# NJU-LHRS/LHRS-Bot

Hardware: AMD Instinct MI355X
Metric: stage-1 pretrain samples/sec (224^2 image + 128-tok caption) (higher is better)
Workload: dtype bf16

## Files before the change

include/lhrs_hip.h:

```cpp
#ifndef LHRS_HIP_H
#define LHRS_HIP_H
#include <stdint.h>
#ifdef __cplusplus
extern "C" {
#endif

typedef uint16_t lhrs_bf16_t;

const char* lhrs_last_error(void);
int lhrs_abi_version(void);
const char* lhrs_target_arch(void);

int lhrs_gemm_bf16_nt(const void* A, int lda, const void* B, int ldb, void* C, int ldc, int M, int N, int K,
                      const void* bias, const void* residual, int ldr, int act, int out_f32, int accumulate,
                      float alpha, void* stream);

int lhrs_gemm_bf16_nt_lora(const void* A, int lda, const void* B, int ldb, const void* A2, int lda2, const void* B2, int ldb2,
                           int K2, void* C, int ldc, int M, int N, int K, const void* bias, const void* residual, int ldr,
                           int out_f32, int accumulate, float alpha, void* stream);
int lhrs_gemm_fp8_nt(const void* A8, long lda, const float* sa, const void* B8, long ldb, const float* sb, void* C, int ldc,
                     int M, int N, int K, const void* residual, int ldr, float alpha, void* stream);
int lhrs_gemm_fp8_nt_lora(const void* A8, long lda, const float* sa, const void* B8, long ldb, const float* sb, const void* A2,
                          int lda2, const void* B2, int ldb2, int K2, void* C, int ldc, int M, int N, int K,
                          const void* residual, int ldr, float alpha, void* stream);
// ... 52 lines not shown
int lhrs_gemm_u4_nt(const void* A, int lda, const void* B, int ldb, void* C, int ldc, int M, int N, int K, const void* residual, int ldr,
                    void* stream);
int lhrs_gemm_u4_nt_lora(const void* A, int lda, const void* B, int ldb, const void* A2, int lda2, const void* B2, int ldb2, int K2, void* C, int ldc,
                         int M, int N, int K, const void* residual, int ldr, void* stream);
int lhrs_gemm_u4_fused_takes(int kind, int M, int tiles_n, int K, int K2);
int lhrs_gemm_u4_main_rows(int M, int N);
int lhrs_gemm_u4_rope(const void* X, int ldx, const void* W, int ldw, void* C, int ldc, int M, int N, int K, const float* cos_t,
                      const float* sin_t, int pos_mod, int pos0, int rope_cols, void* stream);
int lhrs_gemm_u4_rope_lora(const void* X, int ldx, const void* W, int ldw, const void* A2, int lda2, const void* B2, int ldb2, int K2, void* C, int ldc,
                           int M, int N, int K, const float* cos_t, const float* sin_t, int pos_mod, int pos0, int rope_cols, void* stream);
int lhrs_gemm_u4_swiglu_fwd(const void* X, int ldx, const void* Wgu, int ldw, void* gu, int ld_gu, void* act, int ld_act, int M, int ff, int K,
                            void* stream);
int lhrs_gemm_u4_swiglu_bwd(const void* dY, int ldy, const void* WdT, int ldw, const void* gu, void* dgu, int ld_gu, int M, int ff, int K,
                            void* stream);

int lhrs_tn_skinny_splits(int M, int N);
int lhrs_gemm_tn_skinny(const void* P, long ldp, const void* Q, long ldq, float* C, long ldc, float* partial, int M, int N,
                        int KP, int accumulate, void* stream);
int lhrs_blockdiag_mask(float* g, long ld, int rows, int cols, int r, int w, int active_mask, void* stream);

int lhrs_layernorm_fwd(const void* x, long ldx, const void* gamma, const void* beta, void* y, long ldy, float* mean,
                       float* rstd, int rows, int cols, float eps, void* stream);
int lhrs_layernorm_bwd_nblk(int rows);
int lhrs_layernorm_bwd(const void* dy, long ld_dy, const void* x, long ldx, const void* gamma, const float* mean,
                       const float* rstd, const void* add, void* dx, long ld_dx, float* dgamma, float* dbeta,
                       float* partial, int accumulate, int rows, int cols, void* stream);
int lhrs_rmsnorm_fwd(const void* x, long ldx, const void* w, void* y, long ldy, float* rstd, int rows, int cols,
                     float eps, void* stream);
int lhrs_rmsnorm_bwd(const void* dy, const void* x, const void* w, const float* rstd, const void* add, void* dx,
                     int rows, int cols, float eps, void* stream);

int lhrs_seq_transpose(const void* in, long ld_in, void* out, int cols, int LT, const int* desc, int nseq, int use_kv,
                       void* stream);
int lhrs_attn_fwd(const void* q, long ldq, const void* k, long ldk, const void* v, long ldv, void* o, long ldo, float* lse,
                  const int* desc, int nseq, int H, int D, int max_q, int max_kv, int LTq, int causal, float scale,
                  void* stream);
int lhrs_attn_fwd_kmask(const void* q, long ldq, const void* k, long ldk, const void* v, long ldv, void* o, long ldo,
                        float* lse, const int* desc, int nseq, int H, int D, int max_q, int max_kv, int LTq,
                        int causal, float scale, const unsigned char* key_mask, long ld_mask, void* stream);
int lhrs_attn_delta(const void* o, long ldo, const void* dout, long ld_do, float* delta, const int* desc, int nseq, int H,
                    int D, int max_q, int LTq, void* stream);
int lhrs_attn_bwd(const void* q, long ldq, const void* k, long ldk, const void* v, long ldv, const void* dout,
                  long ld_do, const float* lse, const float* delta, void* dq, long ld_dq, void* dk, long ld_dk, void* dv,
                  long ld_dv, const int* desc, int nseq, int H, int D, int max_q, int max_kv, int LTq, int causal,
                  float scale, void* stream);
int lhrs_attn_bwd_rope(const void* q, long ldq, const void* k, long ldk, const void* v, long ldv, const void* dout,
                       long ld_do, const float* lse, const float* delta, void* dq, long ld_dq, void* dk, long ld_dk, void* dv,
                       long ld_dv, const int* desc, int nseq, int H, int D, int max_q, int max_kv, int LTq, int causal,
                       float scale, const float* cos_t, const float* sin_t, int pos_mod, int pos0, long rows, void* stream);
int lhrs_attn_bwd_o(const void* q, long ldq, const void* k, long ldk, const void* v, long ldv, const void* dout, long ld_do,
                    const void* o, long ldo, const float* lse, float* delta, void* dq, long ld_dq, void* dk, long ld_dk, void* dv,
                    long ld_dv, const int* desc, int nseq, int H, int D, int max_q, int max_kv, int LTq, int causal, float scale,
                    const float* cos_t, const float* sin_t, int pos_mod, int pos0, long rows, void* stream);

int lhrs_patchify(const float* rgb, void* out, int B, int img, int P, int KP, void* stream);
int lhrs_vit_assemble(const void* patch, const void* cls, const void* pos, void* out, int B, int NP, int dim,
                      void* stream);
int lhrs_rope(void* x, long ld, int rows, int nheads, int D, const float* cos_t, const float* sin_t, const int* pos_ids,
              int pos_mod, int pos0, int inverse, void* stream);
int lhrs_swiglu_fwd(const void* gate_up, void* act, long rows, int F, void* stream);
int lhrs_swiglu_bwd(const void* dact, const void* gate_up, void* dgate_up, long rows, int F, void* stream);
int lhrs_map(int op, const void* a, const void* b, void* out, long n, void* stream);
int lhrs_colsum_nsplit(int rows);
int lhrs_colsum(const void* x, long ld, float* out, float* partial, int rows, int cols, int accumulate, void* stream);
int lhrs_cast_f32_to_bf16(const float* in, void* out, long n, void* stream);
int lhrs_cast_bf16_to_f32(const void* in, float* out, long n, void* stream);
// ... 98 lines not shown
```

lhrs_bot_amd/csrc/attention.hip:

```cpp
#include "common.h"
#include <type_traits>

namespace {

struct AttnArgs {
  const bf16_t* q; const bf16_t* k; const bf16_t* v; const bf16_t* dout;
  long ldq, ldk, ldv, ldo, ld_do, ld_dq, ld_dk, ld_dv;
  bf16_t* o; bf16_t* dq; bf16_t* dk; bf16_t* dv;
  int LTq;
  float* lse;
  const float* delta;
  const int* desc;
  int H;
  float scale;
  const unsigned char* kmask;
  long ld_kmask;
  const float* rope_cos;
  const float* rope_sin;
  int rope_mod, rope_pos0;
  const bf16_t* o_in;
  long ld_oin;
  float* delta_w;
  int wide;
};

constexpr float NEG_INF = -__builtin_huge_valf();

template <int D>
__device__ __forceinline__ int swz(int row) {
  return D == 128 ? (((row & 7) << 1) | ((row >> 3) & 1)) : (row & 7);
}
template <int D>
__device__ __forceinline__ int rm_off(int row, int c) { return row * (D * 2) + ((c ^ swz<D>(row)) << 4); }

template <int D> struct TileRegs { uint4 v[64 * (D / 8) / 256]; };

template <int D>
__device__ __forceinline__ void tile_load(TileRegs<D>& r, const bf16_t* base, long ld, int row0, int len, int tid) {
  constexpr int CH = D / 8, N = 64 * CH / 256;
#pragma unroll
  for (int i = 0; i < N; ++i) {
    const int idx = tid + i * 256;
    const int gr = min(row0 + idx / CH, len - 1);
    r.v[i] = *reinterpret_cast<const uint4*>(base + (long)gr * ld + (idx % CH) * 8);
  }
}
template <int D>
__device__ __forceinline__ void tile_store(char* lds, const TileRegs<D>& r, int tid) {
  constexpr int CH = D / 8, N = 64 * CH / 256;
#pragma unroll
  for (int i = 0; i < N; ++i) {
    const int idx = tid + i * 256;
    *reinterpret_cast<uint4*>(lds + rm_off<D>(idx / CH, idx % CH)) = r.v[i];
  }
}
template <int D>
// ... 382 lines not shown
#pragma unroll
    for (int db = 0; db < DB; ++db) dk[db] = MFMA(join(blo[db], bhi[db]), d0, dk[db]);
    tr_wait<DB>(alo, ahi);
    tr_issue<D, 1>(tq, blo, bhi);
    __builtin_amdgcn_sched_barrier(0);
#pragma unroll
    for (int db = 0; db < DB; ++db) dv[db] = MFMA(join(alo[db], ahi[db]), p1, dv[db]);
    tr_wait<DB>(blo, bhi);
#pragma unroll
    for (int db = 0; db < DB; ++db) dk[db] = MFMA(join(blo[db], bhi[db]), d1, dk[db]);
  }
  if (key < kv_rows) {
    bf16_t* pk = a.dk + (long)(kv_off + key) * a.ld_dk + h * D + fg * 4;
    bf16_t* pv = a.dv + (long)(kv_off + key) * a.ld_dv + h * D + fg * 4;
#pragma unroll
    for (int db = 0; db < DB; ++db) { store4bf(pk + db * 16, dk[db], 1.f); store4bf(pv + db * 16, dv[db], 1.f); }
  }
}

template <int D> constexpr int res_rows() { return 163840 / (2 * D * 2); }

template <int D>
__device__ __forceinline__ void res_load(char* lds, const bf16_t* base, long ld, int rows, int len, int lane, int wave) {
  constexpr int CH = D / 8, R = 1024 / (D * 2);
  typedef const __attribute__((address_space(1))) void* gp;
  typedef __attribute__((address_space(3))) void* lp;
  for (int r0 = wave * R; r0 < rows; r0 += 8 * R) {
    const int row = r0 + lane / CH;
    const int c = (lane % CH) ^ swz<D>(row);
    const bf16_t* src = base + (long)min(row, len - 1) * ld + c * 8;
    __builtin_amdgcn_global_load_lds((gp)src, (lp)(lds + r0 * (D * 2)), 16, 0, 0);
  }
}
__device__ __forceinline__ int zigzag_group(int p, int wave, int G, bool descending) {
  const int k = p * 8 + ((p & 1) ? 7 - wave : wave);
  if (k >= G) return -1;
  return descending ? G - 1 - k : k;
}

#ifdef ATTN_DIAG
__device__ unsigned long long* g_attn_dbg = nullptr;
__device__ int g_attn_dbg_sel = 0;
#define DIAG_T(slot) do { if (g_attn_dbg && g_attn_dbg_sel == DIAG_KID && lane == 0) g_attn_dbg[((long)(blockIdx.y * gridDim.x + blockIdx.x) * 8 + wave) * 8 + (slot)] = wall_clock64(); } while (0)
#define DIAG_DECL(id) constexpr int DIAG_KID = id; unsigned long long dg_t = 0, dg_acc[3] = {0, 0, 0}; int dg_units = 0
#define DIAG_MARK() do { asm volatile("s_waitcnt vmcnt(0) lgkmcnt(0)" ::: "memory"); dg_t = wall_clock64(); } while (0)
#define DIAG_ACC(k) do { asm volatile("s_waitcnt vmcnt(0) lgkmcnt(0)" ::: "memory"); const unsigned long long t_ = wall_clock64(); dg_acc[k] += t_ - dg_t; dg_t = t_; } while (0)
#define DIAG_UNITS(n) dg_units += (n)
#define DIAG_FLUSH() do { if (g_attn_dbg && g_attn_dbg_sel == DIAG_KID && lane == 0) { unsigned long long* d_ = g_attn_dbg + ((long)(blockIdx.y * gridDim.x + blockIdx.x) * 8 + wave) * 8; d_[2] = dg_acc[0]; d_[3] = dg_acc[1]; d_[5] = dg_acc[2]; d_[6] = dg_units; } } while (0)
#else
#define DIAG_T(slot) do { } while (0)
#define DIAG_DECL(id)
#define DIAG_MARK() do { } while (0)
#define DIAG_ACC(k) do { } while (0)
#define DIAG_UNITS(n) do { } while (0)
#define DIAG_FLUSH() do { } while (0)
#endif

template <int D, bool CAUSAL>
__global__ __launch_bounds__(512, 2) void attn_fwd_res_kernel(AttnArgs a) {
  constexpr int KS = D / 32, DB = D / 16, TILE = 64 * D * 2;
  __shared__ __attribute__((aligned(16))) char smem[163840];
  char* lds_k = smem;
  char* lds_v = smem + res_rows<D>() * D * 2;
  const int seq = blockIdx.y, h = blockIdx.x;
  const int* ds = a.desc + seq * 8;
  const int q_off = ds[0], q_len = ds[1], kv_off = ds[2], kv_len = ds[3], coff = ds[5];
  const int tid = threadIdx.x, lane = tid & 63, fr = lane & 15, fg = lane >> 4;
  const int wave = __builtin_amdgcn_readfirstlane(tid >> 6);
  DIAG_DECL(0);
  DIAG_T(0);
  int kv_need = kv_len;
  if (CAUSAL) kv_need = max(0, min(kv_len, q_len + coff));
  const int rows = ((kv_need + 63) >> 6) << 6;
  if (rows > 0) {
    res_load<D>(lds_k, a.k + (long)kv_off * a.ldk + h * D, a.ldk, rows, kv_len, lane, wave);
    res_load<D>(lds_v, a.v + (long)kv_off * a.ldv + h * D, a.ldv, rows, kv_len, lane, wave);
  }
  asm volatile("s_waitcnt vmcnt(0)" ::: "memory");
  __syncthreads();
  DIAG_T(1);
  TrAddr<D> tv;
  tv.init(lds_v, lane);
  const float c2 = a.scale * 1.4426950408889634f;
  const int G = (q_len + 15) >> 4;
  for (int p = 0;; ++p) {
    const int g = zigzag_group(p, wave, G, CAUSAL);
    if (g < 0) break;
    DIAG_MARK();
    const int qrow = g * 16 + fr;
    const bf16_t* qp = a.q + (long)(q_off + min(qrow, q_len - 1)) * a.ldq + h * D;
    bf16x8 qf[KS];
#pragma unroll
    for (int ks = 0; ks < KS; ++ks) qf[ks] = *reinterpret_cast<const bf16x8*>(qp + ks * 32 + fg * 8);
    DIAG_ACC(0);
    float m = NEG_INF, l = 0.f;
    f32x4 o[DB];
#pragma unroll
    for (int i = 0; i < DB; ++i) o[i] = f32x4{0.f, 0.f, 0.f, 0.f};
    int kv_end = kv_len;
    if (CAUSAL) kv_end = max(0, min(kv_len, min(g * 16 + 16, q_len) + coff));
// ... 45 lines not shown
      m = m_new;
#pragma unroll
      for (int i = 0; i < DB; ++i) o[i] *= alpha;
      const bf16x8 p0 = pack_frag(s[0], s[1]), p1 = pack_frag(s[2], s[3]);
      tr_wait<DB>(v0lo, v0hi);
      tr_issue<D, 1>(tj, v1lo, v1hi);
      __builtin_amdgcn_sched_barrier(0);
#pragma unroll
      for (int db = 0; db < DB; ++db) o[db] = MFMA(join(v0lo[db], v0hi[db]), p0, o[db]);
      tr_wait<DB>(v1lo, v1hi);
#pragma unroll
      for (int db = 0; db < DB; ++db) o[db] = MFMA(join(v1lo[db], v1hi[db]), p1, o[db]);
    }
    DIAG_ACC(1);
    DIAG_UNITS(ntiles);
    l = group_sum(l);
    if (qrow < q_len) {
      const float inv = l > 0.f ? 1.f / l : 0.f;
      bf16_t* op = a.o + (long)(q_off + qrow) * a.ldo + h * D;
      if (a.wide) store_row_wide<DB>(op, o, inv, fg);
      else {
#pragma unroll
        for (int db = 0; db < DB; ++db) store4bf(op + fg * 4 + db * 16, o[db], inv);
      }
      if (a.lse && fg == 0) a.lse[(long)(seq * a.H + h) * a.LTq + qrow] = (l > 0.f) ? m * a.scale + __logf(l) : NEG_INF;
    }
    DIAG_ACC(2);
  }
  DIAG_T(4);
  DIAG_FLUSH();
}

template <int D, bool CAUSAL>
__global__ __launch_bounds__(512, 2) void attn_bwd_dq_res_kernel(AttnArgs a) {
  constexpr int KS = D / 32, DB = D / 16, TILE = 64 * D * 2;
  __shared__ __attribute__((aligned(16))) char smem[163840];
  char* lds_k = smem;
  char* lds_v = smem + res_rows<D>() * D * 2;
  const int seq = blockIdx.y, h = blockIdx.x;
  const int* ds = a.desc + seq * 8;
  const int q_off = ds[0], q_len = ds[1], kv_off = ds[2], kv_len = ds[3], coff = ds[5];
  const int tid = threadIdx.x, lane = tid & 63, fr = lane & 15, fg = lane >> 4;
  const int wave = __builtin_amdgcn_readfirstlane(tid >> 6);
  DIAG_DECL(1);
  DIAG_T(0);
  int kv_need = kv_len;
  if (CAUSAL) kv_need = max(0, min(kv_len, q_len + coff));
  const int rows = ((kv_need + 63) >> 6) << 6;
  if (rows > 0) {
    res_load<D>(lds_k, a.k + (long)kv_off * a.ldk + h * D, a.ldk, rows, kv_len, lane, wave);
    res_load<D>(lds_v, a.v + (long)kv_off * a.ldv + h * D, a.ldv, rows, kv_len, lane, wave);
  }
  asm volatile("s_waitcnt vmcnt(0)" ::: "memory");
  __syncthreads();
  DIAG_T(1);
  TrAddr<D> tk;
  tk.init(lds_k, lane);
  const int G = (q_len + 15) >> 4;
  for (int p = 0;; ++p) {
    const int g = zigzag_group(p, wave, G, CAUSAL);
    if (g < 0) break;
    DIAG_MARK();
    const int qrow = g * 16 + fr;
    const int qrow_c = min(qrow, q_len - 1);
    const bf16_t* qp = a.q + (long)(q_off + qrow_c) * a.ldq + h * D;
    const bf16_t* dop = a.dout + (long)(q_off + qrow_c) * a.ld_do + h * D;
    bf16x8 qf[KS], dof[KS];
#pragma unroll
    for (int ks = 0; ks < KS; ++ks) {
      qf[ks] = *reinterpret_cast<const bf16x8*>(qp + ks * 32 + fg * 8);
      dof[ks] = *reinterpret_cast<const bf16x8*>(dop + ks * 32 + fg * 8);
    }
    const long stat = (long)(seq * a.H + h) * a.LTq + qrow_c;
    float delta_q;
    if (a.o_in != nullptr) {
// ... 57 lines not shown
            s[nb][r] = ok ? pv * (dp[nb][r] - delta_q) : 0.f;
          }
      }
      const bf16x8 d0 = pack_frag(s[0], s[1]), d1 = pack_frag(s[2], s[3]);
      tr_wait<DB>(k0lo, k0hi);
      tr_issue<D, 1>(tj, k1lo, k1hi);
      __builtin_amdgcn_sched_barrier(0);
#pragma unroll
      for (int db = 0; db < DB; ++db) dq[db] = MFMA(join(k0lo[db], k0hi[db]), d0, dq[db]);
      tr_wait<DB>(k1lo, k1hi);
#pragma unroll
      for (int db = 0; db < DB; ++db) dq[db] = MFMA(join(k1lo[db], k1hi[db]), d1, dq[db]);
    }
    DIAG_ACC(1);
    DIAG_UNITS(ntiles);
    if (qrow < q_len) {
#pragma unroll
      for (int db = 0; db < DB; ++db) dq[db] *= a.scale;
      if (a.rope_cos != nullptr) rope_bwd_inplace<DB>(dq, a, (long)q_off + qrow, fg);
      bf16_t* pq = a.dq + (long)(q_off + qrow) * a.ld_dq + h * D;
      if (a.wide) store_row_wide<DB>(pq, dq, 1.f, fg);
      else {
#pragma unroll
        for (int db = 0; db < DB; ++db) store4bf(pq + fg * 4 + db * 16, dq[db], 1.f);
      }
    }
    DIAG_ACC(2);
  }
  DIAG_T(4);
  DIAG_FLUSH();
}

template <int D, bool CAUSAL>
__global__ __launch_bounds__(512, 2) void attn_bwd_dkv_res_kernel(AttnArgs a) {
  constexpr int KS = D / 32, DB = D / 16, TILE = 64 * D * 2;
  __shared__ __attribute__((aligned(16))) char smem[163840];
  char* lds_q = smem;
  char* lds_do = smem + res_rows<D>() * D * 2;
  const int seq = blockIdx.y, h = blockIdx.x;
  const int* ds = a.desc + seq * 8;
  const int q_off = ds[0], q_len = ds[1], kv_off = ds[2], kv_len = ds[3], kv_rows = ds[4], coff = ds[5];
  const int tid = threadIdx.x, lane = tid & 63, fr = lane & 15, fg = lane >> 4;
  const int wave = __builtin_amdgcn_readfirstlane(tid >> 6);
  DIAG_DECL(2);
  DIAG_T(0);
  const int nq_tiles = (q_len + 63) >> 6;
  const bool half_last = nq_tiles > 0 && q_len - (nq_tiles - 1) * 64 <= 32;
  const int rows_alloc = nq_tiles * 64 - (half_last ? 32 : 0);
  float* lds_lse = reinterpret_cast<float*>(smem + rows_alloc * D * 2);
  float* lds_delta = lds_lse + a.LTq;
  const float* lsebase = a.lse + (long)(seq * a.H + h) * a.LTq;
  const float* deltabase = a.delta + (long)(seq * a.H + h) * a.LTq;
  res_load<D>(lds_q, a.q + (long)q_off * a.ldq + h * D, a.ldq, rows_alloc, q_len, lane, wave);
  res_load<D>(lds_do, a.dout + (long)q_off * a.ld_do + h * D, a.ld_do, rows_alloc, q_len, lane, wave);
  for (int t = tid; t < a.LTq; t += 512) { lds_lse[t] = lsebase[t]; lds_delta[t] = deltabase[t]; }
  asm volatile("s_waitcnt vmcnt(0)" ::: "memory");
  __syncthreads();
  DIAG_T(1);
  TrAddr<D> tq, tdo;
  tq.init(lds_q, lane);
  tdo.init(lds_do, lane);
  const int G = (kv_rows + 15) >> 4;
  for (int p = 0;; ++p) {
    const int g = zigzag_group(p, wave, G, !CAUSAL);
    if (g < 0) break;
    DIAG_MARK();
    const int key = g * 16 + fr;
    const int key_c = min(key, kv_rows - 1);
    const bf16_t* kp = a.k + (long)(kv_off + key_c) * a.ldk + h * D;
    const bf16_t* vp = a.v + (long)(kv_off + key_c) * a.ldv + h * D;
    bf16x8 kf[KS], vf[KS];
#pragma unroll
    for (int ks = 0; ks < KS; ++ks) {
      kf[ks] = *reinterpret_cast<const bf16x8*>(kp + ks * 32 + fg * 8);
      vf[ks] = *reinterpret_cast<const bf16x8*>(vp + ks * 32 + fg * 8);
// ... 75 lines not shown
        const bf16x8 p1 = pack_frag(s[2], s[3]), d1 = pack_frag(dp[2], dp[3]);
        tr_issue<D, 1>(tdi, alo, ahi);
        tr_wait<DB>(alo, ahi);
#pragma unroll
        for (int db = 0; db < DB; ++db) dv[db] = MFMA(join(alo[db], ahi[db]), p1, dv[db]);
        __builtin_amdgcn_sched_barrier(0);
        tr_issue<D, 1>(tqi, alo, ahi);
        tr_wait<DB>(alo, ahi);
#pragma unroll
        for (int db = 0; db < DB; ++db) dk[db] = MFMA(join(alo[db], ahi[db]), d1, dk[db]);
        __builtin_amdgcn_sched_barrier(0);
      }
    }
    RopeRow<DB> rr;
    const bool rope = a.rope_cos != nullptr;
    if (rope) rope_row_load<DB>(rr, a, (long)kv_off + key_c, fg);
    DIAG_ACC(1);
    if (key < kv_rows) {
      if (rope) rope_row_apply<DB>(dk, rr);
      bf16_t* pk = a.dk + (long)(kv_off + key) * a.ld_dk + h * D;
      bf16_t* pv = a.dv + (long)(kv_off + key) * a.ld_dv + h * D;
      if (a.wide) { store_row_wide<DB>(pk, dk, 1.f, fg); store_row_wide<DB>(pv, dv, 1.f, fg); }
      else {
#pragma unroll
        for (int db = 0; db < DB; ++db) { store4bf(pk + fg * 4 + db * 16, dk[db], 1.f); store4bf(pv + fg * 4 + db * 16, dv[db], 1.f); }
      }
    }
    DIAG_ACC(2);
  }
  DIAG_T(4);
  DIAG_FLUSH();
}

template <int D>
__global__ void attn_delta_kernel(const bf16_t* __restrict__ o, long ldo, const bf16_t* __restrict__ dout, long ld_do,
                                  float* __restrict__ delta, const int* __restrict__ desc, int H, int LTq) {
  constexpr int TPR = D / 8;
  const int seq = blockIdx.z, h = blockIdx.y;
  const int q_off = desc[seq * 8 + 0], q_len = desc[seq * 8 + 1];
  const int t = blockIdx.x * (256 / TPR) + threadIdx.x / TPR;
  const int c = threadIdx.x % TPR;
  float s = 0.f;
  if (t < q_len) {
    const uint4 a = *reinterpret_cast<const uint4*>(o + (long)(q_off + t) * ldo + h * D + c * 8);
    const uint4 b = *reinterpret_cast<const uint4*>(dout + (long)(q_off + t) * ld_do + h * D + c * 8);
    s = bflo(a.x) * bflo(b.x) + bfhi(a.x) * bfhi(b.x) + bflo(a.y) * bflo(b.y) + bfhi(a.y) * bfhi(b.y) +
        bflo(a.z) * bflo(b.z) + bfhi(a.z) * bfhi(b.z) + bflo(a.w) * bflo(b.w) + bfhi(a.w) * bfhi(b.w);
  }
#pragma unroll
  for (int off = TPR / 2; off > 0; off >>= 1) s += __shfl_xor(s, off, 64);
  if (t < q_len && c == 0) delta[(long)(seq * H + h) * LTq + t] = s;
}

__global__ __launch_bounds__(256) void seq_transpose_kernel(const bf16_t* __restrict__ in, long ld_in, bf16_t* __restrict__ out,
                                                            int cols, int LT, const int* __restrict__ desc, int off_idx,
                                                            int len_idx) {
  __shared__ bf16_t tile[64][66];
  const int seq = blockIdx.z;
  const int off = desc[seq * 8 + off_idx], len = desc[seq * 8 + len_idx];
  const int t0 = blockIdx.x * 64, c0 = blockIdx.y * 64;
  const int tx = threadIdx.x & 63, ty = threadIdx.x >> 6;
  for (int r = ty; r < 64; r += 4) {
    const int t = t0 + r, c = c0 + tx;
    tile[r][tx] = (t < len && c < cols) ? in[(long)(off + t) * ld_in + c] : (bf16_t)0;
  }
  __syncthreads();
  for (int r = ty; r < 64; r += 4) {
    const int c = c0 + r, t = t0 + tx;
    if (c < cols && t < LT) out[((long)seq * cols + c) * LT + t] = tile[tx][r];
  }
}

int check_common(const AttnArgs& a, int D, int nseq, const char* who) {
  LHRS_REQUIRE(D == 64 || D == 128, "%s: head_dim %d unsupported (64 or 128)", who, D);
  LHRS_REQUIRE(nseq > 0 && a.H > 0, "%s: nseq=%d H=%d", who, nseq, a.H);
  LHRS_REQUIRE(a.LTq % 64 == 0, "%s: LTq must be a multiple of 64", who);
  return 0;
}

}

#ifdef ATTN_DIAG
extern "C" int lhrs_attn_set_dbg(void* p, int sel) {
  unsigned long long* v = (unsigned long long*)p;
  if (hipMemcpyToSymbol(HIP_SYMBOL(g_attn_dbg_sel), &sel, sizeof(sel)) != hipSuccess) return -1;
  return hipMemcpyToSymbol(HIP_SYMBOL(g_attn_dbg), &v, sizeof(v)) == hipSuccess ? 0 : -1;
}
#endif
extern "C" int lhrs_seq_transpose(const void* in, long ld_in, void* out, int cols, int LT, const int* desc, int nseq,
                                  int use_kv, void* stream) {
  LHRS_REQUIRE(LT % 64 == 0 && cols > 0 && nseq > 0, "seq_transpose: LT=%d cols=%d nseq=%d", LT, cols, nseq);
  hipLaunchKernelGGL(seq_transpose_kernel, dim3(LT / 64, cdiv(cols, 64), nseq), dim3(256), 0, (hipStream_t)stream,
                     (const bf16_t*)in, ld_in, (bf16_t*)out, cols, LT, desc, use_kv ? 2 : 0, use_kv ? (use_kv == 2 ? 4 : 3) : 1);
  LHRS_CHECK_LAUNCH("seq_transpose");
  return 0;
}

static int attn_fwd_impl(const void* q, long ldq, const void* k, long ldk, const void* v, long ldv, void* o, long ldo,
                         float* lse, const int* desc, int nseq, int H, int D, int max_q, int max_kv, int LTq,
                         int causal, float scale, const unsigned char* key_mask, long ld_mask, void* stream) {
  AttnArgs a; memset(&a, 0, sizeof(a));
  a.kmask = key_mask; a.ld_kmask = ld_mask;
  if (key_mask != nullptr) max_kv = 1 << 30;
  a.q = (const bf16_t*)q; a.ldq = ldq; a.k = (const bf16_t*)k; a.ldk = ldk; a.v = (const bf16_t*)v; a.ldv = ldv;
  a.o = (bf16_t*)o; a.ldo = ldo; a.lse = lse; a.desc = desc; a.H = H; a.LTq = LTq; a.scale = scale;
  a.wide = (ldo % 8 == 0 && (size_t)o % 16 == 0) ? 1 : 0;
  if (check_common(a, D, nseq, "attn_fwd")) return -1;
  const dim3 grid(cdiv(max_q, 64), H, nseq), blk(256);
  hipStream_t s = (hipStream_t)stream;
  if (max_kv > 0 && max_kv <= (D == 128 ? res_rows<128>() : res_rows<64>())) {
    const dim3 rg(H, nseq), rb(512);
    if (D == 128) {
      if (causal) hipLaunchKernelGGL((attn_fwd_res_kernel<128, true>), rg, rb, 0, s, a);
      else hipLaunchKernelGGL((attn_fwd_res_kernel<128, false>), rg, rb, 0, s, a);
    } else {
      if (causal) hipLaunchKernelGGL((attn_fwd_res_kernel<64, true>), rg, rb, 0, s, a);
      else hipLaunchKernelGGL((attn_fwd_res_kernel<64, false>), rg, rb, 0, s, a);
    }
    LHRS_CHECK_LAUNCH("attn_fwd_res");
    return 0;
  }
  if (D == 128) {
    if (causal) hipLaunchKernelGGL((attn_fwd_kernel<128, true>), grid, blk, 0, s, a);
    else hipLaunchKernelGGL((attn_fwd_kernel<128, false>), grid, blk, 0, s, a);
  } else {
    if (causal) hipLaunchKernelGGL((attn_fwd_kernel<64, true>), grid, blk, 0, s, a);
    else hipLaunchKernelGGL((attn_fwd_kernel<64, false>), grid, blk, 0, s, a);
  }
  LHRS_CHECK_LAUNCH("attn_fwd");
  return 0;
}

extern "C" int lhrs_attn_fwd(const void* q, long ldq, const void* k, long ldk, const void* v, long ldv, void* o, long ldo,
                             float* lse, const int* desc, int nseq, int H, int D, int max_q, int max_kv, int LTq,
                             int causal, float scale, void* stream) {
  return attn_fwd_impl(q, ldq, k, ldk, v, ldv, o, ldo, lse, desc, nseq, H, D, max_q, max_kv, LTq, causal, scale, nullptr, 0, stream);
}

extern "C" int lhrs_attn_fwd_kmask(const void* q, long ldq, const void* k, long ldk, const void* v, long ldv, void* o, long ldo,
                                   float* lse, const int* desc, int nseq, int H, int D, int max_q, int max_kv, int LTq,
                                   int causal, float scale, const unsigned char* key_mask, long ld_mask, void* stream) {
  LHRS_REQUIRE(key_mask != nullptr && ld_mask > 0, "attn_fwd_kmask: key_mask=%p ld_mask=%ld", (const void*)key_mask, ld_mask);
  return attn_fwd_impl(q, ldq, k, ldk, v, ldv, o, ldo, lse, desc, nseq, H, D, max_q, max_kv, LTq, causal, scale, key_mask, ld_mask, stream);
}
// ... 11 lines not shown
                       (const bf16_t*)dout, ld_do, delta, desc, H, LTq);
  LHRS_CHECK_LAUNCH("attn_delta");
  return 0;
}

extern "C" int lhrs_rope(void* x, long ld, int rows, int nheads, int D, const float* cos_t, const float* sin_t, const int* pos_ids, int pos_mod,
                         int pos0, int inverse, void* stream);

static int attn_bwd_impl(const void* q, long ldq, const void* k, long ldk, const void* v, long ldv,
                         const void* dout, long ld_do, const float* lse, const float* delta, void* dq, long ld_dq,
                         void* dk, long ld_dk, void* dv, long ld_dv, const int* desc, int nseq, int H, int D,
                         int max_q, int max_kv, int LTq, int causal, float scale, const float* rope_cos, const float* rope_sin,
                         int rope_mod, int rope_pos0, long rope_rows, void* stream, const void* o = nullptr, long ldo = 0) {
  AttnArgs a; memset(&a, 0, sizeof(a));
  if (o != nullptr) {
    const int rmax0 = D == 128 ? res_rows<128>() : res_rows<64>();
    if (max_kv <= rmax0) { a.o_in = (const bf16_t*)o; a.ld_oin = ldo; a.delta_w = const_cast<float*>(delta); }
    else if (lhrs_attn_delta(o, ldo, dout, ld_do, const_cast<float*>(delta), desc, nseq, H, D, max_q, LTq, stream)) return -1;
  }
  const bool rope = rope_cos != nullptr;
  const int rmax_ = D == 128 ? res_rows<128>() : res_rows<64>();
  const bool dkv_fits = max_q <= rmax_ && (long)((max_q + 31) / 32 * 32) * D * 2 + 2L * LTq * 4 <= (long)rmax_ * D * 2;
  const bool fuse_rope = rope && max_kv <= rmax_ && dkv_fits;
  if (fuse_rope) { a.rope_cos = rope_cos; a.rope_sin = rope_sin; a.rope_mod = rope_mod; a.rope_pos0 = rope_pos0; }
  a.q = (const bf16_t*)q; a.ldq = ldq; a.k = (const bf16_t*)k; a.ldk = ldk; a.v = (const bf16_t*)v; a.ldv = ldv;
  a.dout = (const bf16_t*)dout; a.ld_do = ld_do; a.lse = (float*)lse; a.delta = delta;
  a.dq = (bf16_t*)dq; a.ld_dq = ld_dq; a.dk = (bf16_t*)dk; a.ld_dk = ld_dk; a.dv = (bf16_t*)dv; a.ld_dv = ld_dv;
  a.desc = desc; a.H = H; a.LTq = LTq; a.scale = scale;
  a.wide = (ld_dq % 8 == 0 && ld_dk % 8 == 0 && ld_dv % 8 == 0 && ((size_t)dq | (size_t)dk | (size_t)dv) % 16 == 0) ? 1 : 0;
  if (check_common(a, D, nseq, "attn_bwd")) return -1;
  hipStream_t s = (hipStream_t)stream;
  const dim3 gq(cdiv(max_q, 64), H, nseq), gk(cdiv(max_kv, 64), H, nseq), blk(256);
  const int rmax = D == 128 ? res_rows<128>() : res_rows<64>();
  const dim3 rg(H, nseq), rb(512);
  bool dq_done = false, dkv_done = false;
  if (max_kv <= rmax) {
    if (D == 128) { if (causal) hipLaunchKernelGGL((attn_bwd_dq_res_kernel<128, true>), rg, rb, 0, s, a); else hipLaunchKernelGGL((attn_bwd_dq_res_kernel<128, false>), rg, rb, 0, s, a); }
    else { if (causal) hipLaunchKernelGGL((attn_bwd_dq_res_kernel<64, true>), rg, rb, 0, s, a); else hipLaunchKernelGGL((attn_bwd_dq_res_kernel<64, false>), rg, rb, 0, s, a); }
    dq_done = true;
  }
  if (dkv_fits) {
    if (D == 128) { if (causal) hipLaunchKernelGGL((attn_bwd_dkv_res_kernel<128, true>), rg, rb, 0, s, a); else hipLaunchKernelGGL((attn_bwd_dkv_res_kernel<128, false>), rg, rb, 0, s, a); }
    else { if (causal) hipLaunchKernelGGL((attn_bwd_dkv_res_kernel<64, true>), rg, rb, 0, s, a); else hipLaunchKernelGGL((attn_bwd_dkv_res_kernel<64, false>), rg, rb, 0, s, a); }
    dkv_done = true;
  }
  if (dq_done && dkv_done) { LHRS_CHECK_LAUNCH("attn_bwd_res"); return 0; }
#define LAUNCH_TILED(KERN, GRID)                                                                 \
  do {                                                                                           \
    if (D == 128) { if (causal) hipLaunchKernelGGL((KERN<128, true>), GRID, blk, 0, s, a); else hipLaunchKernelGGL((KERN<128, false>), GRID, blk, 0, s, a); } \
    else { if (causal) hipLaunchKernelGGL((KERN<64, true>), GRID, blk, 0, s, a); else hipLaunchKernelGGL((KERN<64, false>), GRID, blk, 0, s, a); }          \
  } while (0)
  if (!dq_done) LAUNCH_TILED(attn_bwd_dq_kernel, gq);
  if (!dkv_done) LAUNCH_TILED(attn_bwd_dkv_kernel, gk);
#undef LAUNCH_TILED
  LHRS_CHECK_LAUNCH("attn_bwd");
  if (rope) {
    if (lhrs_rope(dq, ld_dq, (int)rope_rows, H, D, rope_cos, rope_sin, nullptr, rope_mod, rope_pos0, 1, stream)) return -1;
    if (lhrs_rope(dk, ld_dk, (int)rope_rows, H, D, rope_cos, rope_sin, nullptr, rope_mod, rope_pos0, 1, stream)) return -1;
  }
  return 0;
}

extern "C" int lhrs_attn_bwd(const void* q, long ldq, const void* k, long ldk, const void* v, long ldv,
                             const void* dout, long ld_do, const float* lse, const float* delta, void* dq, long ld_dq,
                             void* dk, long ld_dk, void* dv, long ld_dv, const int* desc, int nseq, int H, int D,
                             int max_q, int max_kv, int LTq, int causal, float scale, void* stream) {
  return attn_bwd_impl(q, ldq, k, ldk, v, ldv, dout, ld_do, lse, delta, dq, ld_dq, dk, ld_dk, dv, ld_dv, desc, nseq, H, D, max_q, max_kv, LTq,
                       causal, scale, nullptr, nullptr, 1, 0, 0, stream);
}

extern "C" int lhrs_attn_bwd_rope(const void* q, long ldq, const void* k, long ldk, const void* v, long ldv,
                                  const void* dout, long ld_do, const float* lse, const float* delta, void* dq, long ld_dq,
                                  void* dk, long ld_dk, void* dv, long ld_dv, const int* desc, int nseq, int H, int D,
                                  int max_q, int max_kv, int LTq, int causal, float scale, const float* cos_t, const float* sin_t,
// ... 16 lines not shown
```

lhrs_bot_amd/kernels.py:

```python
from __future__ import annotations

import ctypes
import os
from typing import Optional

import torch

from . import _lib

ACT_NONE, ACT_QUICK_GELU, ACT_GELU, ACT_SILU = 0, 1, 2, 3
MAP_GELU, MAP_GELU_BWD, MAP_ADD, MAP_QUICK_GELU = 0, 1, 2, 3


def _L():
    return _lib.load()


def _stream() -> int:
    return torch.cuda.current_stream().cuda_stream


def _p(t: Optional[torch.Tensor]) -> Optional[int]:
    return None if t is None else t.data_ptr()

# ... 318 lines not shown
                                 rows, cols, eps, _stream())
    _lib.check(st, "rmsnorm_bwd_q")
    return dx, (d8, sc)


def h2d(t: torch.Tensor, device) -> torch.Tensor:
    if t.is_cuda:
        return t
    return t.pin_memory().to(device, non_blocking=True)


def make_desc(entries, device) -> torch.Tensor:
    rows = []
    for e in entries:
        e = list(e)
        if len(e) == 4:
            e.append(e[3])
        if len(e) == 5:
            e.append(0)
        rows.append(e + [0, 0])
    return h2d(torch.tensor(rows, dtype=torch.int32), device)


def pad64(n: int) -> int:
    return (n + 63) // 64 * 64


def seq_transpose(x, cols, LT, desc, nseq, which: str):
    out = torch.empty((nseq, cols, LT), device=x.device, dtype=torch.bfloat16)
    use = {"q": 0, "kv": 1, "kv_rows": 2}[which]
    st = _L().lhrs_seq_transpose(x.data_ptr(), x.stride(0), out.data_ptr(), cols, LT, desc.data_ptr(), nseq, use, _stream())
    _lib.check(st, "seq_transpose")
    return out


def attn_fwd(q, k, v, o, lse, desc, nseq, H, D, max_q, max_kv, LTq, causal, scale, key_mask=None):
    if key_mask is None:
        st = _L().lhrs_attn_fwd(q.data_ptr(), q.stride(0), k.data_ptr(), k.stride(0), v.data_ptr(), v.stride(0), o.data_ptr(),
                                o.stride(0), _p(lse), desc.data_ptr(), nseq, H, D, max_q, max_kv, LTq, int(causal), float(scale),
                                _stream())
    else:
        assert key_mask.dtype == torch.uint8 and key_mask.dim() == 2 and key_mask.shape[0] == nseq and key_mask.stride(1) == 1
        st = _L().lhrs_attn_fwd_kmask(q.data_ptr(), q.stride(0), k.data_ptr(), k.stride(0), v.data_ptr(), v.stride(0), o.data_ptr(),
                                      o.stride(0), _p(lse), desc.data_ptr(), nseq, H, D, max_q, max_kv, LTq, int(causal),
                                      float(scale), key_mask.data_ptr(), key_mask.stride(0), _stream())
    _lib.check(st, "attn_fwd")


def attn_delta(o, dout, delta, desc, nseq, H, D, max_q, LTq):
    st = _L().lhrs_attn_delta(o.data_ptr(), o.stride(0), dout.data_ptr(), dout.stride(0), delta.data_ptr(), desc.data_ptr(),
                              nseq, H, D, max_q, LTq, _stream())
    _lib.check(st, "attn_delta")


def attn_bwd(q, k, v, dout, lse, delta, dq, dk, dv, desc, nseq, H, D, max_q, max_kv, LTq, causal, scale, rope=None):
    if rope is None:
        st = _L().lhrs_attn_bwd(q.data_ptr(), q.stride(0), k.data_ptr(), k.stride(0), v.data_ptr(), v.stride(0), dout.data_ptr(),
                                dout.stride(0), lse.data_ptr(), delta.data_ptr(), dq.data_ptr(), dq.stride(0), dk.data_ptr(),
                                dk.stride(0), dv.data_ptr(), dv.stride(0), desc.data_ptr(), nseq, H, D, max_q, max_kv, LTq,
                                int(causal), float(scale), _stream())
    else:
        cos_t, sin_t, pos_mod, pos0 = rope
        st = _L().lhrs_attn_bwd_rope(q.data_ptr(), q.stride(0), k.data_ptr(), k.stride(0), v.data_ptr(), v.stride(0), dout.data_ptr(),
                                     dout.stride(0), lse.data_ptr(), delta.data_ptr(), dq.data_ptr(), dq.stride(0), dk.data_ptr(),
                                     dk.stride(0), dv.data_ptr(), dv.stride(0), desc.data_ptr(), nseq, H, D, max_q, max_kv, LTq,
                                     int(causal), float(scale), cos_t.data_ptr(), sin_t.data_ptr(), int(pos_mod), int(pos0), dq.shape[0],
# ... 600 lines not shown
```

Baseline: 169.5.

## Make resident attention kernels persistent with staggered per-block start delays

Converts the resident-K/V attention forward, dQ and dKV kernels from one block per (sequence, head) pair into persistent kernels. Each kernel now launches at most one block per CU and walks the pairs with a grid stride. With the default mode, each block's start is also delayed by a computed sleep proportional to its slot index, to desynchronise global loads into LDS across CUs and reduce bandwidth contention bursts. The costs are the added __syncthreads between pairs, deliberate idle time at kernel start, and hand-tuned period constants that may not match the real per-pair runtime.

```diff
diff --git a/include/lhrs_hip.h b/include/lhrs_hip.h
--- a/include/lhrs_hip.h
+++ b/include/lhrs_hip.h
@@ -108,6 +108,9 @@
 
 int lhrs_seq_transpose(const void* in, long ld_in, void* out, int cols, int LT, const int* desc, int nseq, int use_kv,
                        void* stream);
+int lhrs_attn_set_persistent(int mode);
+int lhrs_attn_walk_rule(int which, int max_q, int max_kv, int D, int causal, int pairs, int cus, int mode, int* grid, int* d);
+int lhrs_attn_start_wait(int b, int d);
 int lhrs_attn_fwd(const void* q, long ldq, const void* k, long ldk, const void* v, long ldv, void* o, long ldo, float* lse,
                   const int* desc, int nseq, int H, int D, int max_q, int max_kv, int LTq, int causal, float scale,
                   void* stream);
diff --git a/lhrs_bot_amd/csrc/attention.hip b/lhrs_bot_amd/csrc/attention.hip
--- a/lhrs_bot_amd/csrc/attention.hip
+++ b/lhrs_bot_amd/csrc/attention.hip
@@ -22,6 +22,7 @@
   long ld_oin;
   float* delta_w;
   int wide;
+  int pairs, start_d;
 };
 
 constexpr float NEG_INF = -__builtin_huge_valf();
@@ -470,6 +471,11 @@
     __builtin_amdgcn_global_load_lds((gp)src, (lp)(lds + r0 * (D * 2)), 16, 0, 0);
   }
 }
+__device__ __forceinline__ int res_tid() {
+  int t = threadIdx.x;
+  asm volatile("" : "+v"(t));
+  return t;
+}
 __device__ __forceinline__ int zigzag_group(int p, int wave, int G, bool descending) {
   const int k = p * 8 + ((p & 1) ? 7 - wave : wave);
   if (k >= G) return -1;
@@ -479,12 +485,12 @@
 #ifdef ATTN_DIAG
 __device__ unsigned long long* g_attn_dbg = nullptr;
 __device__ int g_attn_dbg_sel = 0;
-#define DIAG_T(slot) do { if (g_attn_dbg && g_attn_dbg_sel == DIAG_KID && lane == 0) g_attn_dbg[((long)(blockIdx.y * gridDim.x + blockIdx.x) * 8 + wave) * 8 + (slot)] = wall_clock64(); } while (0)
+#define DIAG_T(slot) do { if (g_attn_dbg && g_attn_dbg_sel == DIAG_KID && lane == 0) g_attn_dbg[((long)(seq * a.H + h) * 8 + wave) * 8 + (slot)] = wall_clock64(); } while (0)
 #define DIAG_DECL(id) constexpr int DIAG_KID = id; unsigned long long dg_t = 0, dg_acc[3] = {0, 0, 0}; int dg_units = 0
 #define DIAG_MARK() do { asm volatile("s_waitcnt vmcnt(0) lgkmcnt(0)" ::: "memory"); dg_t = wall_clock64(); } while (0)
 #define DIAG_ACC(k) do { asm volatile("s_waitcnt vmcnt(0) lgkmcnt(0)" ::: "memory"); const unsigned long long t_ = wall_clock64(); dg_acc[k] += t_ - dg_t; dg_t = t_; } while (0)
 #define DIAG_UNITS(n) dg_units += (n)
-#define DIAG_FLUSH() do { if (g_attn_dbg && g_attn_dbg_sel == DIAG_KID && lane == 0) { unsigned long long* d_ = g_attn_dbg + ((long)(blockIdx.y * gridDim.x + blockIdx.x) * 8 + wave) * 8; d_[2] = dg_acc[0]; d_[3] = dg_acc[1]; d_[5] = dg_acc[2]; d_[6] = dg_units; } } while (0)
+#define DIAG_FLUSH() do { if (g_attn_dbg && g_attn_dbg_sel == DIAG_KID && lane == 0) { unsigned long long* d_ = g_attn_dbg + ((long)(seq * a.H + h) * 8 + wave) * 8; d_[2] = dg_acc[0]; d_[3] = dg_acc[1]; d_[5] = dg_acc[2]; d_[6] = dg_units; } } while (0)
 #else
 #define DIAG_T(slot) do { } while (0)
 #define DIAG_DECL(id)
@@ -495,15 +501,13 @@
 #endif
 
 template <int D, bool CAUSAL>
-__global__ __launch_bounds__(512, 2) void attn_fwd_res_kernel(AttnArgs a) {
+__device__ __forceinline__ void attn_fwd_res_pair(const AttnArgs& a, char* smem, const int seq, const int h) {
   constexpr int KS = D / 32, DB = D / 16, TILE = 64 * D * 2;
-  __shared__ __attribute__((aligned(16))) char smem[163840];
   char* lds_k = smem;
   char* lds_v = smem + res_rows<D>() * D * 2;
-  const int seq = blockIdx.y, h = blockIdx.x;
   const int* ds = a.desc + seq * 8;
   const int q_off = ds[0], q_len = ds[1], kv_off = ds[2], kv_len = ds[3], coff = ds[5];
-  const int tid = threadIdx.x, lane = tid & 63, fr = lane & 15, fg = lane >> 4;
+  const int tid = res_tid(), lane = tid & 63, fr = lane & 15, fg = lane >> 4;
   const int wave = __builtin_amdgcn_readfirstlane(tid >> 6);
   DIAG_DECL(0);
   DIAG_T(0);
@@ -615,15 +619,13 @@
 }
 
 template <int D, bool CAUSAL>
-__global__ __launch_bounds__(512, 2) void attn_bwd_dq_res_kernel(AttnArgs a) {
+__device__ __forceinline__ void attn_bwd_dq_res_pair(const AttnArgs& a, char* smem, const int seq, const int h) {
   constexpr int KS = D / 32, DB = D / 16, TILE = 64 * D * 2;
-  __shared__ __attribute__((aligned(16))) char smem[163840];
   char* lds_k = smem;
   char* lds_v = smem + res_rows<D>() * D * 2;
-  const int seq = blockIdx.y, h = blockIdx.x;
   const int* ds = a.desc + seq * 8;
   const int q_off = ds[0], q_len = ds[1], kv_off = ds[2], kv_len = ds[3], coff = ds[5];
-  const int tid = threadIdx.x, lane = tid & 63, fr = lane & 15, fg = lane >> 4;
+  const int tid = res_tid(), lane = tid & 63, fr = lane & 15, fg = lane >> 4;
   const int wave = __builtin_amdgcn_readfirstlane(tid >> 6);
   DIAG_DECL(1);
   DIAG_T(0);
@@ -747,15 +749,13 @@
 }
 
 template <int D, bool CAUSAL>
-__global__ __launch_bounds__(512, 2) void attn_bwd_dkv_res_kernel(AttnArgs a) {
+__device__ __forceinline__ void attn_bwd_dkv_res_pair(const AttnArgs& a, char* smem, const int seq, const int h) {
   constexpr int KS = D / 32, DB = D / 16, TILE = 64 * D * 2;
-  __shared__ __attribute__((aligned(16))) char smem[163840];
   char* lds_q = smem;
   char* lds_do = smem + res_rows<D>() * D * 2;
-  const int seq = blockIdx.y, h = blockIdx.x;
   const int* ds = a.desc + seq * 8;
   const int q_off = ds[0], q_len = ds[1], kv_off = ds[2], kv_len = ds[3], kv_rows = ds[4], coff = ds[5];
-  const int tid = threadIdx.x, lane = tid & 63, fr = lane & 15, fg = lane >> 4;
+  const int tid = res_tid(), lane = tid & 63, fr = lane & 15, fg = lane >> 4;
   const int wave = __builtin_amdgcn_readfirstlane(tid >> 6);
   DIAG_DECL(2);
   DIAG_T(0);
@@ -897,6 +897,61 @@
   DIAG_FLUSH();
 }
 
+constexpr int ATTN_WAIT_SLEEP = 2;
+constexpr int ATTN_WAIT_UNIT_NS = 60;
+constexpr int ATTN_WAIT_CAP = 667;
+__host__ __device__ __forceinline__ int res_start_wait(int b, int d) {
+  const int n = (b >> 3) * d;
+  return n < ATTN_WAIT_CAP ? n : ATTN_WAIT_CAP;
+}
+#define ATTN_RES_KERNEL(NAME)                                                                                  \
+  template <int D, bool CAUSAL>                                                                                \
+  __global__ __launch_bounds__(512, 2) void NAME##_kernel(AttnArgs a) {                                        \
+    __shared__ __attribute__((aligned(16))) char smem[163840];                                                 \
+    const int b0 = blockIdx.x, step = gridDim.x;                                                               \
+    if (a.start_d > 0)                                                                                         \
+      for (int i = res_start_wait(b0, a.start_d); i > 0; --i) __builtin_amdgcn_s_sleep(ATTN_WAIT_SLEEP);      \
+    for (int pr = b0; pr < a.pairs; pr += step) {                                                              \
+      if (pr != b0) __syncthreads();                                                                           \
+      const int seq = __builtin_amdgcn_readfirstlane(pr / a.H);                                                \
+      NAME##_pair<D, CAUSAL>(a, smem, seq, pr - seq * a.H);                                                    \
+    }                                                                                                          \
+  }
+ATTN_RES_KERNEL(attn_fwd_res)
+ATTN_RES_KERNEL(attn_bwd_dq_res)
+ATTN_RES_KERNEL(attn_bwd_dkv_res)
+#undef ATTN_RES_KERNEL
+
+int g_attn_persist = 2;
+constexpr int ATTN_PERIOD_NS[3] = {280, 430, 500};
+constexpr long ATTN_OFFSET_MIN_IMAGE = 128 << 10;
+void res_walk_rule(int which, int max_q, int max_kv, int D, int causal, int pairs, int cus, int mode, int* grid, int* d) {
+  *grid = (mode == 0 || pairs < cus) ? pairs : cus;
+  *d = 0;
+  if (mode != 2 || which < 0 || which > 2 || *grid <= 8 || pairs < 4 * *grid) return;
+  const int rows = which == 2 ? max_kv : max_q, across = which == 2 ? max_q : max_kv;
+  const long G = cdiv(rows, 16), T = cdiv(across, 64);
+  if (2 * T * 64 * D * 2 < ATTN_OFFSET_MIN_IMAGE) return;
+  const long period_ns = ATTN_PERIOD_NS[which] * G * (causal ? T + 1 : 2 * T) / 2 * D / 128;
+  const int slots = cdiv(*grid, 8);
+  long units = period_ns / slots / ATTN_WAIT_UNIT_NS;
+  if (units < 1) units = 1;
+  if (units * (slots - 1) > ATTN_WAIT_CAP) units = ATTN_WAIT_CAP / (slots - 1);
+  *d = (int)units;
+}
+int res_cus() {
+  int dev = 0, cus = 256;
+  (void)hipGetDevice(&dev);
+  (void)hipDeviceGetAttribute(&cus, hipDeviceAttributeMultiprocessorCount, dev);
+  return cus;
+}
+dim3 res_grid(AttnArgs& a, int which, int nseq, int D, int max_q, int max_kv, int causal) {
+  int grid = 0;
+  a.pairs = nseq * a.H;
+  res_walk_rule(which, max_q, max_kv, D, causal, a.pairs, res_cus(), g_attn_persist, &grid, &a.start_d);
+  return dim3(grid);
+}
+
 template <int D>
 __global__ void attn_delta_kernel(const bf16_t* __restrict__ o, long ldo, const bf16_t* __restrict__ dout, long ld_do,
                                   float* __restrict__ delta, const int* __restrict__ desc, int H, int LTq) {
@@ -952,6 +1007,17 @@
   return hipMemcpyToSymbol(HIP_SYMBOL(g_attn_dbg), &v, sizeof(v)) == hipSuccess ? 0 : -1;
 }
 #endif
+extern "C" int lhrs_attn_set_persistent(int mode) {
+  LHRS_REQUIRE(mode >= 0 && mode <= 2, "attn_set_persistent: mode %d (0 grid of pairs, 1 persistent walk, 2 walk + start offsets)", mode);
+  g_attn_persist = mode;
+  return 0;
+}
+extern "C" int lhrs_attn_walk_rule(int which, int max_q, int max_kv, int D, int causal, int pairs, int cus, int mode, int* grid, int* d) {
+  LHRS_REQUIRE(which >= 0 && which <= 2 && grid && d && pairs > 0 && cus > 0 && max_q > 0 && max_kv > 0, "attn_walk_rule: which=%d pairs=%d cus=%d", which, pairs, cus);
+  res_walk_rule(which, max_q, max_kv, D, causal, pairs, cus, mode, grid, d);
+  return 0;
+}
+extern "C" int lhrs_attn_start_wait(int b, int d) { return res_start_wait(b, d); }
 extern "C" int lhrs_seq_transpose(const void* in, long ld_in, void* out, int cols, int LT, const int* desc, int nseq,
                                   int use_kv, void* stream) {
   LHRS_REQUIRE(LT % 64 == 0 && cols > 0 && nseq > 0, "seq_transpose: LT=%d cols=%d nseq=%d", LT, cols, nseq);
@@ -974,7 +1040,7 @@
   const dim3 grid(cdiv(max_q, 64), H, nseq), blk(256);
   hipStream_t s = (hipStream_t)stream;
   if (max_kv > 0 && max_kv <= (D == 128 ? res_rows<128>() : res_rows<64>())) {
-    const dim3 rg(H, nseq), rb(512);
+    const dim3 rg = res_grid(a, 0, nseq, D, max_q, max_kv, causal), rb(512);
     if (D == 128) {
       if (causal) hipLaunchKernelGGL((attn_fwd_res_kernel<128, true>), rg, rb, 0, s, a);
       else hipLaunchKernelGGL((attn_fwd_res_kernel<128, false>), rg, rb, 0, s, a);
@@ -1052,14 +1118,16 @@
   hipStream_t s = (hipStream_t)stream;
   const dim3 gq(cdiv(max_q, 64), H, nseq), gk(cdiv(max_kv, 64), H, nseq), blk(256);
   const int rmax = D == 128 ? res_rows<128>() : res_rows<64>();
-  const dim3 rg(H, nseq), rb(512);
+  const dim3 rb(512);
   bool dq_done = false, dkv_done = false;
   if (max_kv <= rmax) {
+    const dim3 rg = res_grid(a, 1, nseq, D, max_q, max_kv, causal);
     if (D == 128) { if (causal) hipLaunchKernelGGL((attn_bwd_dq_res_kernel<128, true>), rg, rb, 0, s, a); else hipLaunchKernelGGL((attn_bwd_dq_res_kernel<128, false>), rg, rb, 0, s, a); }
     else { if (causal) hipLaunchKernelGGL((attn_bwd_dq_res_kernel<64, true>), rg, rb, 0, s, a); else hipLaunchKernelGGL((attn_bwd_dq_res_kernel<64, false>), rg, rb, 0, s, a); }
     dq_done = true;
   }
   if (dkv_fits) {
+    const dim3 rg = res_grid(a, 2, nseq, D, max_q, max_kv, causal);
     if (D == 128) { if (causal) hipLaunchKernelGGL((attn_bwd_dkv_res_kernel<128, true>), rg, rb, 0, s, a); else hipLaunchKernelGGL((attn_bwd_dkv_res_kernel<128, false>), rg, rb, 0, s, a); }
     else { if (causal) hipLaunchKernelGGL((attn_bwd_dkv_res_kernel<64, true>), rg, rb, 0, s, a); else hipLaunchKernelGGL((attn_bwd_dkv_res_kernel<64, false>), rg, rb, 0, s, a); }
     dkv_done = true;
diff --git a/lhrs_bot_amd/kernels.py b/lhrs_bot_amd/kernels.py
--- a/lhrs_bot_amd/kernels.py
+++ b/lhrs_bot_amd/kernels.py
@@ -374,6 +374,18 @@
     st = _L().lhrs_seq_transpose(x.data_ptr(), x.stride(0), out.data_ptr(), cols, LT, desc.data_ptr(), nseq, use, _stream())
     _lib.check(st, "seq_transpose")
     return out
+
+
+def attn_set_persistent(mode: int) -> None:
+    _lib.check(_L().lhrs_attn_set_persistent(int(mode)), "attn_set_persistent")
+
+
+def attn_walk_rule(which: int, max_q, max_kv, D, causal, pairs, cus=256, mode=2):
+    import ctypes
+    g, d = ctypes.c_int(0), ctypes.c_int(0)
+    _lib.check(_L().lhrs_attn_walk_rule(int(which), int(max_q), int(max_kv), int(D), int(bool(causal)), int(pairs), int(cus), int(mode), ctypes.byref(g), ctypes.byref(d)),
+               "attn_walk_rule")
+    return g.value, d.value
 
 
 def attn_fwd(q, k, v, o, lse, desc, nseq, H, D, max_q, max_kv, LTq, causal, scale, key_mask=None):
```

Result: no change. 169.9, median of 6 (+0.2%).
